# MiNeves00/SR-GAN-FD

Hardware: AMD Instinct MI355X
Metric: SR training images/sec (128->512 x4, f16) (higher is better)
Workload: dtype f16; 1 GPU; BSRGAN RRDBNet x4 generator-only (L1), 23 RRDB, batch 32/GPU, 128->512; global_batch=32, num_rrdb=23, parallelism=dp1

## Files before the change

sr_gan_fd_amd/csrc/conv_igemm.hip:

```cpp
#include "conv_common.hpp"
#include <stdlib.h>
#include <string.h>
#include <utility>
#ifndef SRGANFD_CROSS_MASK
#define SRGANFD_CROSS_MASK 7
#endif
#ifndef SRGANFD_M16_PIPE
#define SRGANFD_M16_PIPE 4
#endif

namespace srganfd {
typedef __attribute__((ext_vector_type(2))) unsigned int u32x2_t;

template <typename T, int KS, int STRIDE, int MR, int WR, int WN, int TS = 1>
struct ConvCfg {
  static constexpr int NWAVES = WR * WN, NTHR = 64 * NWAVES;
  static constexpr int KT = KS * KS;
  static constexpr int TW = 32, TH = WR * MR;
  static constexpr int PR = (TH - 1) * STRIDE + KS;
  static constexpr int PC = (TW - 1) * STRIDE + KS;
  static constexpr int KC = 32;
  static constexpr int E16 = 16 / (int)sizeof(T);
  static constexpr int CPP = KC / E16;
  static constexpr int PIXB = KC * (int)sizeof(T);
// ... 672 lines not shown

template <typename T, int KS, int STRIDE, int MR, int WR, int WN, bool M16 = false, int TS = 1, int EK = -1, bool NT = false>
static int launch_conv(const ConvK& k, int cout, hipStream_t stream) {
  using C = ConvCfg<T, KS, STRIDE, MR, WR, WN, TS>;
  auto kern = conv_igemm_kernel<T, KS, STRIDE, MR, WR, WN, M16, TS, EK, NT>;
  if (g_describe) {
    char ek[8] = "";
    if (EK >= 0) snprintf(ek, sizeof(ek), ",E%d", EK);
    snprintf(g_describe, g_describe_len, "conv_igemm_kernel<%s,KS=%d,S=%d,MR=%d,WR=%d,WN=%d%s%s%s>%s", dtype_name<T>(), KS, STRIDE, MR, WR, WN, M16 ? ",M16" : "", TS > 1 ? ",TS=2" : "", ek,
             k.cls_sh >= 0 ? "[4 classes]" : "");
    return SRGANFD_OK;
  }
  static unsigned long long attr_done = 0;
  if (!g_dry_run) {
    int dev = 0;
    SRGANFD_HIP_CHECK(hipGetDevice(&dev));
    if (!(attr_done >> (dev & 63) & 1ULL)) {
      SRGANFD_HIP_CHECK(hipFuncSetAttribute((const void*)kern, hipFuncAttributeMaxDynamicSharedMemorySize, C::LDS_BYTES));
      attr_done |= 1ULL << (dev & 63);
    }
  }
  ConvK kk = k;
  kk.nNb = cout / C::NB;
  if (k.cls_sh >= 0) {
    if ((KS != 2 && KS != 1) || STRIDE != 1 || sizeof(T) != 2 || (kk.nNb & (kk.nNb - 1)))
      return set_err(SRGANFD_EINVAL, "conv2d: out_classes needs ksize 2 or 1, stride 1 and cout / %d a power of two", C::NB);
    kk.cls_sh = __builtin_ctz((unsigned)kk.nNb);
    kk.nNb *= 4;
  }
  kk.tiles_x = ceil_div(k.Wout, C::TW);
  kk.tiles_y = ceil_div(k.Hout, C::TH);
  const long long nblk = (long long)k.N * kk.tiles_x * kk.tiles_y * kk.nNb;
  if (nblk <= 0 || nblk > 0x7fffffffLL) return set_err(SRGANFD_EINVAL, "conv2d: bad grid %lld", nblk);
  kk.nblocks = (int)nblk;
  kk.m_nNb = div_magic((unsigned)kk.nNb, (unsigned long long)nblk);
  kk.m_tx = div_magic((unsigned)kk.tiles_x, (unsigned long long)nblk);
  kk.m_ty = div_magic((unsigned)kk.tiles_y, (unsigned long long)nblk);
  long long grid = nblk;
  if (EK >= 0 && (EK & SRGANFD_CROSS_MASK) == 0 && sizeof(T) == 2) {
    const long long slots = (long long)conv_device_cus() * C::WG_PER_CU;
    if (slots >= 8 && nblk > slots) grid = slots / 8 * 8;
  }
  SRGANFD_LAUNCH(kern, dim3((unsigned)grid), dim3(C::NTHR), C::LDS_BYTES, stream, kk);
  SRGANFD_HIP_CHECK(hipGetLastError());
  return SRGANFD_OK;
}



int g_mfma16 = 3;
static const bool g_conv_nt = [] { const char* e = getenv("SRGANFD_CONV_NT"); return !(e && e[0] == '0'); }();

bool conv_uses_m16(int dtype, int ksize, int cout) {
  (void)ksize; (void)cout;
  return dtype != SRGANFD_F32;
}

template <typename T>
static int dispatch_conv(const srganfd_conv_args* a, const ConvK& k, hipStream_t s) {
  const bool wide = (a->cout % 64) == 0;
  constexpr bool bf = sizeof(T) == 2;
  if constexpr (bf) {
    if (conv_uses_m16(a->dtype, a->ksize, a->cout)) {
      if (a->ksize == 3 && a->stride == 1) {
        const int ek = (k.fast_epi && !k.y2) ? ((k.r1 ? 1 : 0) | (k.r2 ? 2 : 0) | (k.mask ? 4 : 0)) : -1;
        if (wide) {
          const size_t opix_ = (size_t)a->n * (size_t)k.HoutF * (size_t)k.WoutF;
          if (g_conv_nt && opix_ * (size_t)a->cout_store * 2 >= ((size_t)192 << 20)) {
            if (ek == 0) return launch_conv<T, 3, 1, 2, 4, 2, true, 1, 0, true>(k, a->cout, s);
            if (ek == 4) return launch_conv<T, 3, 1, 2, 4, 2, true, 1, 4, true>(k, a->cout, s);
            if (ek < 0) return launch_conv<T, 3, 1, 2, 4, 2, true, 1, -1, true>(k, a->cout, s);
          }
          if (ek == 0) return launch_conv<T, 3, 1, 2, 4, 2, true, 1, 0>(k, a->cout, s);
          if (ek == 1) return launch_conv<T, 3, 1, 2, 4, 2, true, 1, 1>(k, a->cout, s);
          if (ek == 3) return launch_conv<T, 3, 1, 2, 4, 2, true, 1, 3>(k, a->cout, s);
          if (ek == 4) return launch_conv<T, 3, 1, 2, 4, 2, true, 1, 4>(k, a->cout, s);
          return launch_conv<T, 3, 1, 2, 4, 2, true>(k, a->cout, s);
        }
        if (ek == 0) return launch_conv<T, 3, 1, 2, 8, 1, true, 1, 0>(k, a->cout, s);
        if (ek == 4) return launch_conv<T, 3, 1, 2, 8, 1, true, 1, 4>(k, a->cout, s);
        return launch_conv<T, 3, 1, 2, 8, 1, true>(k, a->cout, s);
      }
      if (a->ksize == 3 && a->stride == 2) return wide ? launch_conv<T, 3, 2, 1, 4, 2, true>(k, a->cout, s) : launch_conv<T, 3, 2, 1, 4, 1, true>(k, a->cout, s);
      if (a->ksize == 2 && a->stride == 1) return wide ? launch_conv<T, 2, 1, 2, 4, 2, true>(k, a->cout, s) : launch_conv<T, 2, 1, 2, 8, 1, true>(k, a->cout, s);
      if (a->ksize == 4 && a->stride == 2) return wide ? launch_conv<T, 4, 2, 1, 4, 2, true, 2>(k, a->cout, s) : launch_conv<T, 4, 2, 1, 4, 1, true>(k, a->cout, s);
      if (a->ksize == 2 && a->stride == 2) return wide ? launch_conv<T, 2, 2, 1, 4, 2, true>(k, a->cout, s) : launch_conv<T, 2, 2, 1, 4, 1, true>(k, a->cout, s);
      if (a->ksize == 1 && a->stride == 1) return launch_conv<T, 1, 1, 2, 4, 1, true>(k, a->cout, s);
      return set_err(SRGANFD_EINVAL, "conv2d: unsupported ksize=%d stride=%d", a->ksize, a->stride);
    }
  }
  if constexpr (bf) {
    return set_err(SRGANFD_EINVAL, "conv2d: the 16-bit kernels run on v_mfma_f32_16x16x32 (ksize %d stride %d has no kernel)", a->ksize, a->stride);
  } else {
    if (a->ksize == 3 && a->stride == 1) return wide ? launch_conv<T, 3, 1, 2, 4, 2>(k, a->cout, s) : launch_conv<T, 3, 1, 2, 8, 1>(k, a->cout, s);
    if (a->ksize == 2 && a->stride == 1) return wide ? launch_conv<T, 2, 1, 2, 4, 2>(k, a->cout, s) : launch_conv<T, 2, 1, 2, 8, 1>(k, a->cout, s);
    if (a->ksize == 4 && a->stride == 2) return launch_conv<T, 4, 2, 1, 4, 1>(k, a->cout, s);
    if (a->ksize == 3 && a->stride == 2) return wide ? launch_conv<T, 3, 2, 1, 4, 2>(k, a->cout, s) : launch_conv<T, 3, 2, 1, 4, 1>(k, a->cout, s);
    if (a->ksize == 2 && a->stride == 2) return wide ? launch_conv<T, 2, 2, 1, 4, 2>(k, a->cout, s) : launch_conv<T, 2, 2, 1, 4, 1>(k, a->cout, s);
    if (a->ksize == 1 && a->stride == 1) return launch_conv<T, 1, 1, 2, 4, 1>(k, a->cout, s);
    return set_err(SRGANFD_EINVAL, "conv2d: unsupported ksize=%d stride=%d", a->ksize, a->stride);
  }
}

int conv_fill_k(const srganfd_conv_args* a, ConvK& k) {
  if (!a || !a->x.ptr || !a->y.ptr || !a->w_packed) return set_err(SRGANFD_EINVAL, "conv2d: null pointer");
  if (a->cin <= 0 || a->cin % 32 || a->cout <= 0 || a->cout % 32 || a->cout_store <= 0 || a->cout_store > a->cout)
    return set_err(SRGANFD_EINVAL, "conv2d: cin=%d cout=%d cout_store=%d (need multiples of 32)", a->cin, a->cout, a->cout_store);
  if (a->n <= 0 || a->h_in <= 0 || a->w_in <= 0 || a->h_out <= 0 || a->w_out <= 0)
    return set_err(SRGANFD_EINVAL, "conv2d: bad dims");
  const int hl = a->h_in << (a->up ? 1 : 0), wl = a->w_in << (a->up ? 1 : 0);
  const bool sub = a->out_sy > 1 || a->out_sx > 1;
  const bool allcls = a->out_classes == 4;
  if (a->out_classes != 0 && a->out_classes != 1 && !allcls) return set_err(SRGANFD_EINVAL, "conv2d: out_classes is 0, 1 or 4");
  if (allcls && (a->out_sy != 2 || a->out_sx != 2 || (a->ksize != 2 && a->ksize != 1) || a->stride != 1 || a->dtype == SRGANFD_F32 || a->up ||
                 (a->class_pad_step != 0 && a->class_pad_step != 1)))
    return set_err(SRGANFD_EINVAL, "conv2d: out_classes = 4 is the 16-bit data gradient of a stride-2 conv (ksize 2 or 1, stride 1, out_sy = out_sx = 2, class_pad_step 0 / 1)");
  if (!sub) {
    const int ho = (hl + 2 * a->pad - a->ksize) / a->stride + 1, wo = (wl + 2 * a->pad - a->ksize) / a->stride + 1;
    if (ho != a->h_out || wo != a->w_out)
      return set_err(SRGANFD_EINVAL, "conv2d: h_out/w_out %dx%d inconsistent with input (expect %dx%d)", a->h_out, a->w_out, ho, wo);
  } else if (a->out_h_full < (a->h_out - 1) * a->out_sy + (allcls ? 1 : a->out_oy) + 1 || a->out_w_full < (a->w_out - 1) * a->out_sx + (allcls ? 1 : a->out_ox) + 1) {
    return set_err(SRGANFD_EINVAL, "conv2d: strided output does not fit the full image");
  }
  const int align = a->dtype == SRGANFD_F32 ? 4 : 8;
  if (a->x.cstride % align || a->x.c0 % align) return set_err(SRGANFD_EINVAL, "conv2d: x view not 16-byte aligned");
  if (a->x.c0 + a->cin > a->x.cstride) return set_err(SRGANFD_EINVAL, "conv2d: x view exceeds buffer channels");
  if (a->y.c0 + a->cout_store > a->y.cstride) return set_err(SRGANFD_EINVAL, "conv2d: y view exceeds buffer channels");
  if ((size_t)a->h_in * a->w_in * (size_t)a->x.cstride >= 0x7fffffffULL)
    return set_err(SRGANFD_EINVAL, "conv2d: one input image is too large for 32-bit element offsets");
  if (a->dtype != SRGANFD_F32 && (size_t)a->h_in * a->w_in * (size_t)a->x.cstride * 2 >= 0x7fffffffULL)
    return set_err(SRGANFD_EINVAL, "conv2d: one input image exceeds the 2 GiB a buffer descriptor's range check can separate from padding");
  const size_t opix = sub ? (size_t)a->out_h_full * a->out_w_full : (size_t)a->h_out * a->w_out;
  auto fits = [&](const srganfd_view& v) { return !v.ptr || opix * (size_t)v.cstride < 0x7fffffffULL; };
  if (!fits(a->y) || !fits(a->y2) || !fits(a->r1) || !fits(a->r2) || !fits(a->mask))
    return set_err(SRGANFD_EINVAL, "conv2d: one output-side image is too large for 32-bit element offsets");
  k.x = a->x.ptr; k.y = a->y.ptr; k.y2 = a->y2.ptr; k.y2C = a->y2.cstride; k.y2_c0 = a->y2.c0;
  k.r1 = a->r1.ptr; k.r2 = a->r2.ptr; k.mask = a->mask.ptr; k.w = a->w_packed;
  k.bias = a->bias; k.alpha_dev = a->alpha_dev;
  k.xC = a->x.cstride; k.x_c0 = a->x.c0; k.yC = a->y.cstride; k.y_c0 = a->y.c0;
  k.r1C = a->r1.cstride; k.r1_c0 = a->r1.c0; k.r2C = a->r2.cstride; k.r2_c0 = a->r2.c0;
  k.mC = a->mask.cstride; k.m_c0 = a->mask.c0;
  {
    const long long ipix = (long long)a->h_in * a->w_in;
    for (const srganfd_view* v : {&a->x, &a->y, &a->y2, &a->r1, &a->r2, &a->mask})
      if (v->ptr && v->planar && (v->c0 % 32 || v->cstride % 32)) return set_err(SRGANFD_EINVAL, "conv2d: a planar view needs c0 and cstride multiples of 32");
    if (a->y.planar && a->y_f32) return set_err(SRGANFD_EINVAL, "conv2d: fp32 output views are NHWC only");
    k.x_ps = a->x.planar ? 32 : a->x.cstride;
    k.x_cs = a->x.planar ? (int)(ipix * 32) : 32;
    k.x_base = a->x.planar ? (a->x.c0 / 32) * k.x_cs : a->x.c0;
    auto out_strides = [&](const srganfd_view& v, int& ps, int& gs) { ps = v.planar ? 32 : v.cstride; gs = v.planar ? (int)(opix * 32) : 32; };
    out_strides(a->y, k.y_ps, k.y_gs); out_strides(a->y2, k.y2_ps, k.y2_gs); out_strides(a->r1, k.r1_ps, k.r1_gs);
    out_strides(a->r2, k.r2_ps, k.r2_gs); out_strides(a->mask, k.m_ps, k.m_gs);
  }
  k.N = a->n; k.Hin = a->h_in; k.Win = a->w_in; k.up = a->up ? 1 : 0; k.pad_y = sub ? a->pad_y : a->pad; k.pad_x = sub ? a->pad_x : a->pad;
  k.osy = sub ? a->out_sy : 1; k.osx = sub ? a->out_sx : 1; k.ooy = sub ? a->out_oy : 0; k.oox = sub ? a->out_ox : 0;
  k.HoutF = sub ? a->out_h_full : a->h_out; k.WoutF = sub ? a->out_w_full : a->w_out;
  k.Hout = a->h_out; k.Wout = a->w_out; k.nChunks = a->cin / 32; k.nNb = 0; k.cls_sh = allcls ? 0 : -1; k.cls_pad = allcls ? a->class_pad_step : 0; k.cout_store = a->cout_store;
  k.tiles_x = k.tiles_y = 0;
  k.alpha = a->alpha; k.slope = a->slope; k.post_scale = a->post_scale; k.r1s = a->r1_scale; k.r2s = a->r2_scale;
  k.mask_slope = a->mask_slope; k.act = a->act; k.y_f32 = a->y_f32 ? 1 : 0;
  auto aligned = [&](const srganfd_view& v) { return !v.ptr || (v.cstride % align == 0 && v.c0 % align == 0 && ((uintptr_t)v.ptr & 15) == 0); };
  k.fast_epi = (!a->y_f32 && a->cout_store == a->cout && aligned(a->y) && aligned(a->y2) && aligned(a->r1) && aligned(a->r2) && aligned(a->mask)) ? 1 : 0;
  return SRGANFD_OK;
}

int conv2d_impl(const srganfd_conv_args* a, hipStream_t stream) {
  ConvK k;
  {
    const int rc = conv_fill_k(a, k);
    if (rc != SRGANFD_OK) return rc;
  }
  if (a->dtype == SRGANFD_BF16) return dispatch_conv<bf16_t>(a, k, stream);
  if (a->dtype == SRGANFD_F16) return dispatch_conv<f16_t>(a, k, stream);
  if (a->dtype == SRGANFD_F32) return dispatch_conv<float>(a, k, stream);
  return set_err(SRGANFD_EINVAL, "conv2d: bad dtype %d", a->dtype);
}

}
```

sr_gan_fd_amd/csrc/pack.hip:

```cpp
#include "common.hpp"

namespace srganfd {

__global__ __launch_bounds__(256) void pack_kernel(const srganfd_pack_job* __restrict__ jobs, const float* __restrict__ params,
                                                   const float* __restrict__ scalars, char* __restrict__ packed) {
  const srganfd_pack_job& J = jobs[blockIdx.y];
  const int KT = J.ksize * J.ksize;
  const long long total = (long long)KT * J.k * J.n;
  const int nChunks = J.k >> 5;
  for (long long e = (long long)blockIdx.x * 256 + threadIdx.x; e < total; e += (long long)gridDim.x * 256) {
    int lane, s, k_in, within = (int)(e & 1023);
    long long blk = e >> 10;
    const int tap = (int)(blk % KT); blk /= KT;
    const int chunk = (int)(blk % nChunks);
    const int ntile = (int)(blk / nChunks);
    int n_in = -1;
    if (J.dtype != SRGANFD_F32 && J.layout == 1) {
      const int j = within & 7; lane = (within >> 3) & 63; s = within >> 9;
      k_in = 8 * (lane >> 4) + j;
      n_in = 16 * s + (lane & 15);
    } else if (J.dtype != SRGANFD_F32) {
      const int j = within & 7; lane = (within >> 3) & 63; s = within >> 9;
      k_in = 16 * s + 8 * (lane >> 5) + j;
    } else {
      lane = within & 63; s = within >> 6;
      k_in = 2 * s + (lane >> 5);
    }
    const int k = chunk * 32 + k_in, n = ntile * 32 + (n_in >= 0 ? n_in : (lane & 31));
    float v = 0.f;
    for (int g = 0; g < J.nseg; ++g) {
      const srganfd_pack_seg& S = J.seg[g];
      if (k >= S.k_lo && k < S.k_lo + S.k_len) {
        const int kk = k - S.k_lo;
        int co, ci, t;
        int KTs = KT;
        if (!S.transposed) { co = n + S.co_off; ci = kk + S.ci_off; t = tap; }
        else if (S.transposed == 1) { co = kk + S.co_off; ci = n + S.ci_off; t = KT - 1 - tap; }
        else if (S.transposed < 6) {
          const int py = (S.transposed - 2) >> 1, px = (S.transposed - 2) & 1, ta = tap >> 1, tb = tap & 1;
          const int ty = py ? 2 - 2 * ta : 3 - 2 * ta, tx = px ? 2 - 2 * tb : 3 - 2 * tb;
          co = kk + S.co_off; ci = n + S.ci_off; t = ty * 4 + tx; KTs = 16;
        } else if (S.transposed < 10) {
          const int py = (S.transposed - 6) >> 1, px = (S.transposed - 6) & 1, ta = tap >> 1, tb = tap & 1;
          const int ty = py ? (ta ? 0 : 2) : (ta ? -1 : 1), tx = px ? (tb ? 0 : 2) : (tb ? -1 : 1);
          co = kk + S.co_off; ci = n + S.ci_off; KTs = 9;
          t = ty * 3 + tx;
          if (ty < 0 || tx < 0) co = S.co_src;
        } else {
          const int ab = S.transposed - 10;
          co = kk + S.co_off; ci = n + S.ci_off; t = ab; KTs = 4;
        }
        if (co < S.co_src && ci < S.ci_src) {
          v = params[S.src_off + ((long long)co * S.ci_src + ci) * KTs + t] * S.scale;
          if (S.scale_off >= 0) v *= scalars[S.scale_off];
        }
        break;
      }
    }
    if (J.dtype == SRGANFD_BF16) ((bf16_t*)(packed + J.dst_off))[e] = f2bf(v);
    else if (J.dtype == SRGANFD_F16) ((f16_t*)(packed + J.dst_off))[e] = (f16_t)v;
    else ((float*)(packed + J.dst_off))[e] = v;
  }
}

int pack_weights_impl(const srganfd_pack_job* jobs_dev, int njobs, long long max_elems, const float* params,
                      const float* scalars, void* packed, hipStream_t stream) {
  if (!jobs_dev || njobs <= 0 || max_elems <= 0 || !params || !packed) return set_err(SRGANFD_EINVAL, "pack_weights: bad args");
  long long gx = (max_elems + 255) / 256;
  if (gx > 4096) gx = 4096;
  SRGANFD_LAUNCH(pack_kernel, dim3((unsigned)gx, (unsigned)njobs), dim3(256), 0, stream, jobs_dev, params, scalars, (char*)packed);
  SRGANFD_HIP_CHECK(hipGetLastError());
  return SRGANFD_OK;
}

}
```

sr_gan_fd_amd/engine.py:

```python
from __future__ import annotations

import ctypes as C
import os
import weakref
from typing import Dict, List, Optional, Sequence, Tuple

import torch
from torch import Tensor, nn

from . import _abi as A
from . import ops
from . import profiling

_ENGINES: "weakref.WeakKeyDictionary[nn.Module, object]" = weakref.WeakKeyDictionary()


def _require_gpu(x: Tensor) -> None:
    if not x.is_cuda and not A.DRY_RUN:
        raise A.SrganfdError("sr_gan_fd_amd runs on MI355X only: input tensor is not on a GPU (no CPU fallback)")
    A.lib()


def check_channels(what: str, x: Tensor, channels: int) -> None:
    if x.dim() != 4 or x.shape[1] != channels:
# ... 50 lines not shown
                for p, o, n, s in zip(self.params, self.offsets, self.numels, self.shapes):
                    f[o:o + n].copy_(p.detach().reshape(-1).to(device=device, dtype=torch.float32))
                    p.data = f[o:o + n].view(s)
            self.flat = f
            self.version += 1
        return f

    def touch(self) -> None:
        self.version += 1

    def signature(self) -> tuple:
        return (self.flat.data_ptr(), self.flat._version, self.version, tuple(p._version for p in self.params))

    def stale(self, pk: dict) -> bool:
        sig = self.signature()
        if pk.get("seen") != sig:
            pk["seen"] = sig
            return True
        return False

    def new_grad(self, device) -> Tensor:
        if self.total == sum(self.numels):
            return torch.empty(self.total, dtype=torch.float32, device=device)
        return torch.zeros(self.total, dtype=torch.float32, device=device)

    def grad_views(self, flat_grad: Tensor) -> List[Tensor]:
        return [flat_grad[o:o + n].view(s) for o, n, s in zip(self.offsets, self.numels, self.shapes)]


class _Shape:
    pass


class PlanCache:

    def __init__(self, cap: int = 8, cap_pinned: int = 2):
        from collections import OrderedDict
        self.d: "OrderedDict[tuple, tuple]" = OrderedDict()
        self.cap, self.cap_pinned = cap, cap_pinned

    def get(self, key):
        v = self.d.get(key)
        if v is None:
            return None
        self.d.move_to_end(key)
        return v[0]

    def put(self, key, sp, pinned: bool = False) -> None:
        self.d[key] = (sp, pinned)
        self.d.move_to_end(key)
        for want_pinned, cap in ((False, self.cap), (True, self.cap_pinned)):
            keys = [k for k, (_, pin) in self.d.items() if pin == want_pinned]
            for k in keys[:max(0, len(keys) - cap)]:
                del self.d[k]

    def __setitem__(self, key, sp) -> None:
        self.put(key, sp)

    def __len__(self) -> int:
        return len(self.d)

    def __contains__(self, key) -> bool:
        return key in self.d

    def clear(self) -> None:
        self.d.clear()


class TrunkEngine:

    def __init__(self, owner: nn.Module, rdbs: Sequence[nn.Module], rrdb: bool, full: bool):
        self.owner = owner
        self.rdbs = list(rdbs)
        self.rrdb = rrdb
        self.full = full
        self.R = len(self.rdbs)
        c5 = self.rdbs[0].conv5.weight
        self.Cc = c5.shape[0]
        self.G = self.rdbs[0].conv1.weight.shape[0]
        if self.Cc % 32 or self.G % 32:
            raise A.SrganfdError("channels and growth_channels must be multiples of 32 for the MFMA path")
        self.Ccat = self.Cc + 4 * self.G
        self.unshuffle = 1
        if full:
            self.n_up = owner.n_upsample()
            self.in_ch = owner.conv1.weight.shape[1]
            self.out_ch = owner.conv4.weight.shape[0]
            self.unshuffle = getattr(owner, "unshuffle", 1)
        self.fp = FlatParams(list(owner.named_parameters()))
        self.shapes = PlanCache()
        self.packed: Dict[int, dict] = {}
        self.token = 0
        self._rdb_prefix = self._find_prefixes()

    def _find_prefixes(self) -> List[str]:
        names = {id(m): n for n, m in self.owner.named_modules()}
        out = []
        for r in self.rdbs:
            n = names[id(r)]
            out.append(n + "." if n else "")
        return out

    def _poff(self, name: str) -> int:
        return self.fp.off(name)

    def _build_pack(self, dtc: int, device) -> dict:
        Cc, G, Ccat = self.Cc, self.G, self.Ccat
        jobs, offs, cur = [], {}, 0

        def add(key, ksize, k, n, segs):
            nonlocal cur
            offs[key] = cur
            jobs.append(ops.pack_job(cur, dtc, ksize, k, n, segs))
            cur += (ops.packed_bytes(dtc, ksize, k, n) + 255) // 256 * 256

        def fwd(key, wname, co, ci):
            add(key, 3, ops.pad32(ci), ops.pad32(co), [dict(src_off=self._poff(wname), co_src=co, ci_src=ci, k_len=ops.pad32(ci))])

        def bwd(key, wname, co, ci):
            add(key, 3, ops.pad32(co), ops.pad32(ci), [dict(src_off=self._poff(wname), co_src=co, ci_src=ci, k_len=ops.pad32(co), transposed=1)])

        for i, pre in enumerate(self._rdb_prefix):
            for k in range(1, 6):
                cin, cout = Cc + (k - 1) * G, (Cc if k == 5 else G)
                fwd(("f", i, k), f"{pre}conv{k}.weight", cout, cin)
            s5 = 0.2 * (0.2 if (self.rrdb and i % 3 == 2) else 1.0)
            dyoff = {5: 0, 4: Cc, 3: Cc + G, 2: Cc + 2 * G, 1: Cc + 3 * G}
            for step in range(5):
                c_lo = Cc + (3 - step) * G if step < 4 else 0
                n = G if step < 4 else Cc
                kdim = Cc + step * G
                segs = []
                for j in range(5, 4 - step, -1):
                    cin_j, cout_j = Cc + (j - 1) * G, (Cc if j == 5 else G)
                    segs.append(dict(src_off=self._poff(f"{pre}conv{j}.weight"), co_src=cout_j, ci_src=cin_j, k_lo=dyoff[j],
                                     k_len=cout_j, ci_off=c_lo, transposed=1, scale=(s5 if j == 5 else 1.0)))
                add(("b", i, step), 3, kdim, n, segs)
        if self.full:
            fwd(("f", "conv1"), "conv1.weight", Cc, self.in_ch)
            for nm in ["conv2"] + [f"upsampling{u}.0" for u in range(1, self.n_up + 1)] + ["conv3.0"]:
                fwd(("f", nm), nm + ".weight", Cc, Cc)
                bwd(("b", nm), nm + ".weight", Cc, Cc)
            fwd(("f", "conv4"), "conv4.weight", self.out_ch, Cc)
            bwd(("b", "conv4"), "conv4.weight", self.out_ch, Cc)
        table = ops.PackTable(jobs, device)
        buf = torch.empty(cur, dtype=torch.uint8, device=device)
        return dict(table=table, offs=offs, buf=buf)

    def _ensure_packed(self, dtc: int, device) -> dict:
        flat = self.fp.sync(device)
        pk = self.packed.get(dtc)
        if pk is None or pk["buf"].device != device or pk.get("flat_ptr") != flat.data_ptr():
            pk = self._build_pack(dtc, device)
            pk["flat_ptr"] = flat.data_ptr()
            self.packed[dtc] = pk
        if self.fp.stale(pk):
            pk["table"].run(flat, pk["buf"])
        return pk

    def _plan(self, N: int, H: int, W: int, dt: torch.dtype, dtc: int, device, train: bool, pk: dict) -> _Shape:
        key = (N, H, W, dtc, train, str(device), pk["buf"].data_ptr(), self.fp.flat.data_ptr())
        sp = self.shapes.get(key)
        if sp is not None:
            return sp
        sp = _Shape()
        Cc, G, Ccat, R = self.Cc, self.G, self.Ccat, self.R
        flat = self.fp.flat
        fptr = flat.data_ptr()
        wptr = pk["buf"].data_ptr()

        def new(*shape, dtype=dt):
            return torch.empty(*shape, dtype=dtype, device=device)

        if train:
            cat = sp.cat = [new(N, H, W, Ccat) for _ in range(R + 1)]
            catb = lambda i: cat[i]
        else:
            cat = sp.cat = [new(N, H, W, Ccat) for _ in range(min(R + 1, 5))]
            catb = lambda i: cat[0] if i == 0 else cat[1 + (i - 1) % 4]
        sp.catb = catb
        V = A.view
        sp.planar = 1 if (self.full and os.environ.get("SRGANFD_PLANAR", "1") != "0") else 0
        VC = lambda t, c0=0: A.view(t, c0=c0, planar=sp.planar)

        def bias(name):
            return fptr + 4 * self._poff(name)

        fw = []
        if self.full:
            s = 1 << self.n_up
            sp.thin_i, sp.thin_o = ops.thin_ok(dtc, Cc, self.in_ch), ops.thin_ok(dtc, Cc, self.out_ch)
            cin1 = ops.pad32(self.in_ch)
            sp.xin = new(N, H, W, 4 if sp.thin_i else cin1)
            sp.f0 = new(N, H, W, Cc)
            sp.ups = [new(N, H << u, W << u, Cc) for u in range(1, self.n_up + 1)]
            sp.c3 = new(N, H * s, W * s, Cc)
            sp.srp = new(N, H * s, W * s, 4, dtype=torch.float32)
            if sp.thin_i:
                fw.append(ops.ThinLaunch("thin_in", ops.thin_args(dtc, N, H, W, self.in_ch, bias("conv1.weight"), VC(catb(0)), w_big_is_cout=True,
                                                                  bias=bias("conv1.bias"), thin=sp.xin)))
            else:
                fw.append(ops.conv_args(dtc, V(sp.xin), VC(catb(0)), wptr + pk["offs"][("f", "conv1")], N, H, W, cin1, Cc, bias=bias("conv1.bias")))
        for i, pre in enumerate(self._rdb_prefix):
            ci = catb(i)
            blk = []
            for k in range(1, 5):
                blk.append(ops.conv_args(dtc, VC(ci), VC(ci, c0=Cc + (k - 1) * G), wptr + pk["offs"][("f", i, k)], N, H, W, Cc + (k - 1) * G, G,
                                         bias=bias(f"{pre}conv{k}.bias"), act=A.ACT_LRELU, slope=0.2))
            last = self.rrdb and i % 3 == 2
            kw = dict(post_scale=0.04, r1=VC(ci), r1_scale=0.2, r2=VC(catb(i - 2)), r2_scale=1.0) if last else \
                dict(post_scale=0.2, r1=VC(ci), r1_scale=1.0)
            blk.append(ops.conv_args(dtc, VC(ci), VC(catb(i + 1)), wptr + pk["offs"][("f", i, 5)], N, H, W, Ccat, Cc,
                                     bias=bias(f"{pre}conv5.bias"), **kw))
            fw.extend(ops.dense_chain_or_launches(blk, device) if (Cc, G) == (64, 32) else blk)
        if self.full:
            tout = catb(R)
            fw.append(ops.conv_args(dtc, VC(tout), V(sp.f0), wptr + pk["offs"][("f", "conv2")], N, H, W, Cc, Cc, bias=bias("conv2.bias"),
                                    r1=VC(catb(0)), r1_scale=1.0))
            src, h, w = sp.f0, H, W
            for u in range(1, self.n_up + 1):
                nm = f"upsampling{u}.0"
                fw.append(ops.conv_args(dtc, V(src), V(sp.ups[u - 1]), wptr + pk["offs"][("f", nm)], N, h, w, Cc, Cc, up=1,
                                        bias=bias(nm + ".bias"), act=A.ACT_LRELU, slope=0.2))
                src, h, w = sp.ups[u - 1], h * 2, w * 2
            fw.append(ops.conv_args(dtc, V(src), V(sp.c3), wptr + pk["offs"][("f", "conv3.0")], N, h, w, Cc, Cc, bias=bias("conv3.0.bias"),
                                    act=A.ACT_LRELU, slope=0.2))
            if sp.thin_o:
                fw.append(ops.ThinLaunch("thin_out", ops.thin_args(dtc, N, h, w, self.out_ch, bias("conv4.weight"), V(sp.c3), w_big_is_cout=False,
                                                                   bias=bias("conv4.bias"), thin_out=sp.srp, thin_out_pitch=4)))
            else:
                fw.append(ops.conv_args(dtc, V(sp.c3), V(sp.srp), wptr + pk["offs"][("f", "conv4")], N, h, w, Cc, 32, cout_store=self.out_ch,
                                        bias=bias("conv4.bias"), y_f32=True))
            sp.hs, sp.ws = h, w
        sp.fw = fw
        sp.N, sp.H, sp.W, sp.dt, sp.dtc, sp.device = N, H, W, dt, dtc, device
        if train:
            self._plan_backward(sp, pk)
        self.shapes.put(key, sp, pinned=train)
        return sp

    def _plan_backward(self, sp: _Shape, pk: dict) -> None:
        N, H, W, dt, dtc, device = sp.N, sp.H, sp.W, sp.dt, sp.dtc, sp.device
        Cc, G, Ccat, R = self.Cc, self.G, self.Ccat, self.R
        wptr = pk["buf"].data_ptr()
        V = A.view
        VC = lambda t, c0=0: A.view(t, c0=c0, planar=sp.planar)
        VD = VC

        def new(*shape, dtype=dt):
            return torch.empty(*shape, dtype=dtype, device=device)

        sp.dy = [new(N, H, W, Ccat) for _ in range(4)]
        sp.dx0 = new(N, H, W, Cc)
        dyb = lambda i: sp.dy[i % 4]
        bw: List[tuple] = []
        ws_bytes = 0

        def wplan(n, h, w, xch, dych, convs, up=0):
            nonlocal ws_bytes
            p = ops.WgradPlan(device, dtc, n, h, w, xch, dych, convs, up=up)
            ws_bytes = max(ws_bytes, p.workspace_bytes)
            return p

        if self.full:
            s = 1 << self.n_up
            hs, ws_ = sp.hs, sp.ws
            sp.dsrp = new(N, hs, ws_, 4 if sp.thin_o else 32)
            sp.gA = new(N, hs, ws_, Cc)
            fptr = self.fp.flat.data_ptr()
            if sp.thin_i or sp.thin_o:
                sp.thin_ws = torch.empty(ops.thin_wgrad_workspace_bytes(), dtype=torch.uint8, device=device)
            sp.gB = new(N, hs, ws_, Cc)
            sp.glo = [new(N, H << u, W << u, Cc) for u in range(0, self.n_up)]

            def one(name, cout, cin, dw_only=False):
                return [dict(cin=ops.pad32(cin), cout=ops.pad32(cout), dw_off=self._poff(name + ".weight"), db_off=self._poff(name + ".bias"),
                             co_dst=cout, ci_dst=cin)]
            if sp.thin_o:
                w4 = fptr + 4 * self._poff("conv4.weight")
                bw.append(("thin", ops.ThinLaunch("thin_wgrad", ops.thin_args(dtc, N, hs, ws_, self.out_ch, w4, V(sp.c3), w_big_is_cout=False, thin=sp.dsrp),
                                                  dw_off=self._poff("conv4.weight"), db_off=self._poff("conv4.bias"), ws=sp.thin_ws)))
                bw.append(("thin", ops.ThinLaunch("thin_in", ops.thin_args(dtc, N, hs, ws_, self.out_ch, w4, V(sp.gA), w_big_is_cout=False, flip=True,
                                                                           mask=V(sp.c3), mask_slope=0.2, thin=sp.dsrp))))
            else:
                bw.append(("wgrad", wplan(N, hs, ws_, Cc, 32, one("conv4", self.out_ch, Cc)), V(sp.c3), V(sp.dsrp), 0))
                bw.append(("conv", ops.conv_args(dtc, V(sp.dsrp), V(sp.gA), wptr + pk["offs"][("b", "conv4")], N, hs, ws_, 32, Cc, mask=V(sp.c3), mask_slope=0.2)))
            src3 = sp.ups[-1] if self.n_up else sp.f0
            bw.append(("wgrad", wplan(N, hs, ws_, Cc, Cc, one("conv3.0", Cc, Cc)), V(src3), V(sp.gA), 0))
            if self.n_up:
                bw.append(("conv", ops.conv_args(dtc, V(sp.gA), V(sp.gB), wptr + pk["offs"][("b", "conv3.0")], N, hs, ws_, Cc, Cc, mask=V(src3), mask_slope=0.2)))
            else:
                bw.append(("conv", ops.conv_args(dtc, V(sp.gA), V(sp.gB), wptr + pk["offs"][("b", "conv3.0")], N, hs, ws_, Cc, Cc)))
            cur, other = sp.gB, sp.gA
            for u in range(self.n_up, 0, -1):
                nm = f"upsampling{u}.0"
                hin, win = H << (u - 1), W << (u - 1)
                xin_t = sp.ups[u - 2] if u >= 2 else sp.f0
                npx = N * (hin * 2) * (win * 2)
                cur_v = V(cur.view(-1)[: npx * Cc].view(N, hin * 2, win * 2, Cc))
                oth_v = V(other.view(-1)[: npx * Cc].view(N, hin * 2, win * 2, Cc))
                bw.append(("wgrad", wplan(N, hin, win, Cc, Cc, one(nm, Cc, Cc), up=1), V(xin_t), cur_v, 0))
                bw.append(("conv", ops.conv_args(dtc, cur_v, oth_v, wptr + pk["offs"][("b", nm)], N, hin * 2, win * 2, Cc, Cc)))
                glo = sp.glo[u - 1]
                bw.append(("call", (lambda a=oth_v, b=V(glo), hh=hin, ww=win: A.check(
                    A.lib().srganfd_resample(0, a, b, dtc, N, hh, ww, Cc, A.stream_ptr()), "nearest_bwd"))))
                if u >= 2:
                    bw.append(("call", (lambda d=V(glo), act=V(xin_t), npx2=N * hin * win: A.check(
                        A.lib().srganfd_lrelu_bwd(d, act, A.NULL_VIEW, d, dtc, npx2, Cc, 0.2, A.stream_ptr()), "lrelu_bwd"))))
                    cur, other = glo, sp.gA
                else:
                    cur = glo
            d_f0 = cur if self.n_up else sp.gB
            sp.d_f0 = d_f0
            bw.append(("wgrad", wplan(N, H, W, Cc, Cc, one("conv2", Cc, Cc)), VC(sp.catb(R)), V(d_f0), 0))
            bw.append(("conv", ops.conv_args(dtc, V(d_f0), VD(dyb(R - 1)), wptr + pk["offs"][("b", "conv2")], N, H, W, Cc, Cc)))
            bw.append(("ready", self._poff("conv2.weight"), self.fp.total))
        rdb_names = ["conv%d" % k for k in range(1, 6)]
        plans = {}
        for i in range(R - 1, -1, -1):
            pre = self._rdb_prefix[i]
            last = self.rrdb and i % 3 == 2
            first = self.rrdb and i % 3 == 0
            s_out = 0.2 if last else 1.0
            s5 = 0.2 * s_out
            ci, di = sp.catb(i), dyb(i)
            if s5 not in plans:
                base = self._poff(pre + "conv1.weight")
                convs = []
                for k in range(1, 6):
                    cin, cout = Cc + (k - 1) * G, (Cc if k == 5 else G)
                    convs.append(dict(ci_lo=0, cin=cin, co_lo=(0 if k == 5 else Cc + (4 - k) * G), cout=cout,
                                      dw_off=self._poff(pre + f"conv{k}.weight") - base, db_off=self._poff(pre + f"conv{k}.bias") - base,
                                      co_dst=cout, ci_dst=cin, alpha=(s5 if k == 5 else 1.0)))
                plans[s5] = wplan(N, H, W, Ccat, Ccat, convs)
            blk = []
            for step in range(4):
                kdim = Cc + step * G
                blk.append(ops.conv_args(dtc, VD(di), VD(di, c0=Cc + step * G), wptr + pk["offs"][("b", i, step)], N, H, W, kdim, G,
                                         mask=VC(ci, c0=Cc + (3 - step) * G), mask_slope=0.2))
            dst = VD(dyb(i - 1)) if i > 0 else V(sp.dx0)
            kw = dict(r1=VD(di), r1_scale=s_out)
            if first:
                kw.update(r2=VD(dyb(i + 2)), r2_scale=1.0)
            blk.append(ops.conv_args(dtc, VD(di), dst, wptr + pk["offs"][("b", i, 4)], N, H, W, Ccat, Cc, **kw))
            chain = ops.dense_chain_or_launches(blk, sp.device) if (Cc, G) == (64, 32) else blk
            wg = ("wgrad", plans[s5], VC(ci), VD(di), self._poff(pre + "conv1.weight"), i)
            fence = [("fence", i + 3)] if i > 0 else []
            ready = [("ready", self._poff(pre + "conv1.weight"), self._poff("conv2.weight"))] if self.full and R >= 4 and i == R // 2 else []
            if len(chain) == 1:
                bw.extend(fence + [("chain", chain[0]), wg] + ready)
            else:
                bw.extend([("conv", a_) for a_ in blk[:4]] + [wg] + ready + fence + [("conv", blk[4])])
        if self.full:
            bw.append(("call", (lambda x=V(sp.d_f0), y=V(sp.dx0): A.check(
                A.lib().srganfd_axpby(x, y, dtc, N * H * W, Cc, 1.0, 1.0, A.stream_ptr()), "axpby"))))
            if sp.thin_i:
                bw.append(("thin", ops.ThinLaunch("thin_wgrad", ops.thin_args(dtc, N, H, W, self.in_ch, self.fp.flat.data_ptr() + 4 * self._poff("conv1.weight"),
                                                                              V(sp.dx0), w_big_is_cout=True, thin=sp.xin),
                                                  dw_off=self._poff("conv1.weight"), db_off=self._poff("conv1.bias"), ws=sp.thin_ws)))
            else:
                cin1 = ops.pad32(self.in_ch)
                convs = [dict(cin=cin1, cout=Cc, dw_off=self._poff("conv1.weight"), db_off=self._poff("conv1.bias"), co_dst=Cc, ci_dst=self.in_ch)]
                bw.append(("wgrad", wplan(N, H, W, cin1, Cc, convs), V(sp.xin), V(sp.dx0), 0))
        covered = min([it[1] for it in bw if it[0] == "ready"], default=self.fp.total)
        bw.append(("ready", 0, covered))
        sp.bw = bw
        sp.wg_ws = torch.empty(ws_bytes, dtype=torch.uint8, device=device)
        dense_ws = max((p_.workspace_bytes for p_ in plans.values()), default=0)
        sp.wg_ws4 = [torch.empty(dense_ws, dtype=torch.uint8, device=device) for _ in range(_BATCH_REDUCE)] if (dense_ws and _BATCH_REDUCE > 1) else None

    def trunk_size(self, shape) -> Tuple[int, int, int]:
        shape = tuple(shape)
        u = self.unshuffle
        want_c = self.in_ch // (u * u) if self.full else self.Cc
        what = "generator" if self.full else "dense block"
        if len(shape) != 4:
            raise A.SrganfdError(f"{what} expects a 4-D (N, {want_c}, H, W) input, got shape {shape}")
        N, c, H, W = shape
        if c != want_c:
            raise A.SrganfdError(f"{what} expects (N, {want_c}, H, W) inputs, got shape {shape}")
        if H % u or W % u:
            raise A.SrganfdError(f"generator with PixelUnshuffle({u}) expects H and W divisible by {u}: (N, {want_c}, {u}k, {u}m), "
                                 f"got shape {shape}")
        return N, H // u, W // u

    def output_shape(self, shape) -> Tuple[int, int, int, int]:
        N, H, W = self.trunk_size(shape)
        if not self.full:
            return (N, self.Cc, H, W)
        return (N, self.out_ch, H << self.n_up, W << self.n_up)

# ... 213 lines not shown
```

sr_gan_fd_amd/profiling.py:

```python
from __future__ import annotations

from typing import Dict, List, Optional

import torch

REC: Optional["Recorder"] = None


class Recorder:

    def __init__(self, every: int = 7):
        self.items: List[tuple] = []
        self.every = max(1, every)
        self.count: Dict[str, int] = {}
        self.work: Dict[str, list] = {}

    def bracket(self, label: str, work, fn) -> None:
        flops, nbytes = work if isinstance(work, tuple) else (work, 0.0)
        n = self.count.get(label, 0)
        self.count[label] = n + 1
        w = self.work.setdefault(label, [0.0, 0.0])
        w[0] += flops
        w[1] += nbytes
        if n % self.every:
            fn()
            return
        e0, e1 = torch.cuda.Event(enable_timing=True), torch.cuda.Event(enable_timing=True)
        e0.record()
        fn()
        e1.record()
        self.items.append((label, flops, nbytes, e0, e1))


def enable(every: int = 7) -> Recorder:
    global REC
    REC = Recorder(every)
    return REC


def disable() -> None:
    global REC
    REC = None


def conv_label(a) -> str:
    lab = getattr(a, "_kernel_label", None)
    if lab is None:
        import ctypes as C
        from . import _abi as A
        buf = C.create_string_buffer(160)
        A.check(A.lib().srganfd_conv2d_describe(C.byref(a), buf, 160), "conv2d_describe")
        lab = a._kernel_label = buf.value.decode()
    return lab


def conv_flops(a) -> float:
    return 2.0 * a.n * a.h_out * a.w_out * a.ksize * a.ksize * a.cin * a.cout_store * (4 if a.out_classes == 4 else 1)


def conv_work(a) -> tuple:
    es = 4 if a.dtype == 1 else 2
    pin = a.n * a.h_in * a.w_in * a.cin * es
    pout = a.n * a.h_out * a.w_out * a.cout_store * (4 if a.out_classes == 4 else 1)
    nb = pin + pout * (4 if a.y_f32 else es)
    for v in (a.r1, a.r2, a.mask, a.y2):
        if v.ptr:
            nb += pout * es
    return conv_flops(a), float(nb)


def summary(rec: Recorder) -> Dict[str, dict]:
    torch.cuda.synchronize()
    agg: Dict[str, dict] = {}
    for label, flops, nbytes, e0, e1 in rec.items:
        d = agg.setdefault(label, {"launches": 0, "ms": 0.0, "flop": 0.0, "bytes": 0.0, "timed_launches": 0})
        d["timed_launches"] += 1
        d["ms"] += e0.elapsed_time(e1)
        d["flop"] += flops
        d["bytes"] += nbytes
    for label, d in agg.items():
        d["launches"] = rec.count[label]
    for d in agg.values():
        d["avg_us"] = round(d["ms"] * 1e3 / d["timed_launches"], 2)
        d["tflops"] = round(d["flop"] / (d["ms"] * 1e-3) / 1e12, 1) if d["ms"] > 0 else 0.0
        d["gbps"] = round(d["bytes"] / (d["ms"] * 1e-3) / 1e9, 1) if d["ms"] > 0 else 0.0
        d["flop_per_byte"] = round(d["flop"] / d["bytes"], 1) if d["bytes"] > 0 else None
        scale = d["launches"] / d["timed_launches"]
        d["ms"] = round(d["ms"] * scale, 3)
    for label, d in agg.items():
        d["flop"] = float(f"{rec.work[label][0]:.6g}")
        d["bytes"] = float(f"{rec.work[label][1]:.6g}")
    return agg


MEASURED_READ_GBPS = 5600.0


def roofline(rec: Recorder, peak_tflops: float, peak_gbps: float = 8000.0) -> dict:
    import re
    per_label = summary(rec)
    agg: Dict[str, dict] = {}
    for lab, v in per_label.items():
        fam = re.sub(r",E\d+", "", lab)
        d = agg.setdefault(fam, {"launches": 0, "ms": 0.0, "flop": 0.0, "bytes": 0.0, "kinds": {}})
        d["launches"] += v["launches"]; d["ms"] += v["ms"]; d["flop"] += v["flop"]; d["bytes"] += v["bytes"]
        d["kinds"][lab] = {"launches": v["launches"], "avg_us": v["avg_us"]}
    for d in agg.values():
        d["avg_us"] = round(d["ms"] * 1e3 / d["launches"], 2) if d["launches"] else 0.0
        d["tflops"] = round(d["flop"] / (d["ms"] * 1e-3) / 1e12, 1) if d["ms"] > 0 else 0.0
        d["gbps"] = round(d["bytes"] / (d["ms"] * 1e-3) / 1e9, 1) if d["ms"] > 0 else 0.0
        d["flop_per_byte"] = round(d["flop"] / d["bytes"], 1) if d["bytes"] > 0 else None
    label, d = max(agg.items(), key=lambda kv: kv[1]["ms"])
    ridge = peak_tflops * 1e12 / (peak_gbps * 1e9)
    ai = d["flop_per_byte"]
    hbm = ai is not None and ai < ridge
    out = {"bound": "hbm" if hbm else "mfma", "kernel": label}
    if hbm:
        out.update(achieved=d["gbps"], peak=peak_gbps, unit="GB/s", frac=round(d["gbps"] / peak_gbps, 4))
    else:
        out.update(achieved=d["tflops"], peak=peak_tflops, unit="TFLOP/s", frac=round(d["tflops"] / peak_tflops, 4))
    if len(d["kinds"]) > 1:
        out["kinds"] = d["kinds"]
    slab, sv = max(per_label.items(), key=lambda kv: kv[1]["ms"])
    tot_ms = sum(v["ms"] for v in per_label.values())
    out["largest_symbol"] = {"kernel": slab, "avg_us": sv["avg_us"], "launches": sv["launches"], "tflops": sv["tflops"],
                             "mfma_frac": round(sv["tflops"] / peak_tflops, 4), "share_of_bracketed_kernel_time": round(sv["ms"] / tot_ms, 4) if tot_ms > 0 else None}
    out.update(traffic=None, avg_launch_us=d["avg_us"], launches=d["launches"],
               flop_per_launch=float(f"{d['flop'] / d['launches']:.6g}"),
               bytes_per_launch=float(f"{d['bytes'] / d['launches']:.6g}"), flop_per_byte=ai, ridge_flop_per_byte=round(ridge, 1),
               mfma_frac=round(d["tflops"] / peak_tflops, 4), hbm_frac=round(d["gbps"] / peak_gbps, 4),
               hbm_measured_read_gbps=MEASURED_READ_GBPS, hbm_frac_of_measured=round(d["gbps"] / MEASURED_READ_GBPS, 4))
    return out
```

Before: 539.6 img/s.

## Fold nearest-x2 upsample into parity-decomposed 2x2 convs and 4x4 stride-2 dgrad

Replaces each nearest-x2 upsample followed by a 3x3 conv with four sub-pixel 2x2 convs, whose weights are summed at pack time from the 3x3 taps for each output parity. Where possible these run as a single out_classes=4 launch that works on the low-resolution input. The backward data gradient becomes one 4x4 stride-2 conv with folded weights and a fused leaky-ReLU mask, replacing the conv, nearest-resample reduction and lrelu_bwd kernels. A non-temporal-store variant of the 2x2 kernel is added for large outputs. This removes the 2.25x redundant MACs of convolving the upsampled image and several full-resolution memory passes, at the cost of new pack modes and layout complexity.

```diff
diff --git a/sr_gan_fd_amd/csrc/conv_igemm.hip b/sr_gan_fd_amd/csrc/conv_igemm.hip
--- a/sr_gan_fd_amd/csrc/conv_igemm.hip
+++ b/sr_gan_fd_amd/csrc/conv_igemm.hip
@@ -778,7 +778,11 @@
         return launch_conv<T, 3, 1, 2, 8, 1, true>(k, a->cout, s);
       }
       if (a->ksize == 3 && a->stride == 2) return wide ? launch_conv<T, 3, 2, 1, 4, 2, true>(k, a->cout, s) : launch_conv<T, 3, 2, 1, 4, 1, true>(k, a->cout, s);
-      if (a->ksize == 2 && a->stride == 1) return wide ? launch_conv<T, 2, 1, 2, 4, 2, true>(k, a->cout, s) : launch_conv<T, 2, 1, 2, 8, 1, true>(k, a->cout, s);
+      if (a->ksize == 2 && a->stride == 1) {
+        if (wide && g_conv_nt && k.cls_sh >= 0 && a->bias && (size_t)a->n * (size_t)k.HoutF * (size_t)k.WoutF * (size_t)a->cout_store * 2 >= ((size_t)192 << 20))
+          return launch_conv<T, 2, 1, 2, 4, 2, true, 1, -1, true>(k, a->cout, s);
+        return wide ? launch_conv<T, 2, 1, 2, 4, 2, true>(k, a->cout, s) : launch_conv<T, 2, 1, 2, 8, 1, true>(k, a->cout, s);
+      }
       if (a->ksize == 4 && a->stride == 2) return wide ? launch_conv<T, 4, 2, 1, 4, 2, true, 2>(k, a->cout, s) : launch_conv<T, 4, 2, 1, 4, 1, true>(k, a->cout, s);
       if (a->ksize == 2 && a->stride == 2) return wide ? launch_conv<T, 2, 2, 1, 4, 2, true>(k, a->cout, s) : launch_conv<T, 2, 2, 1, 4, 1, true>(k, a->cout, s);
       if (a->ksize == 1 && a->stride == 1) return launch_conv<T, 1, 1, 2, 4, 1, true>(k, a->cout, s);
@@ -810,7 +814,8 @@
   if (a->out_classes != 0 && a->out_classes != 1 && !allcls) return set_err(SRGANFD_EINVAL, "conv2d: out_classes is 0, 1 or 4");
   if (allcls && (a->out_sy != 2 || a->out_sx != 2 || (a->ksize != 2 && a->ksize != 1) || a->stride != 1 || a->dtype == SRGANFD_F32 || a->up ||
                  (a->class_pad_step != 0 && a->class_pad_step != 1)))
-    return set_err(SRGANFD_EINVAL, "conv2d: out_classes = 4 is the 16-bit data gradient of a stride-2 conv (ksize 2 or 1, stride 1, out_sy = out_sx = 2, class_pad_step 0 / 1)");
+    return set_err(SRGANFD_EINVAL, "conv2d: out_classes = 4 is the 16-bit data gradient of a stride-2 conv or the forward of a nearest-x2 + 3x3 conv "
+                                   "(ksize 2 or 1, stride 1, up 0, out_sy = out_sx = 2, class_pad_step 0 / 1)");
   if (!sub) {
     const int ho = (hl + 2 * a->pad - a->ksize) / a->stride + 1, wo = (wl + 2 * a->pad - a->ksize) / a->stride + 1;
     if (ho != a->h_out || wo != a->w_out)
diff --git a/sr_gan_fd_amd/csrc/pack.hip b/sr_gan_fd_amd/csrc/pack.hip
--- a/sr_gan_fd_amd/csrc/pack.hip
+++ b/sr_gan_fd_amd/csrc/pack.hip
@@ -32,8 +32,9 @@
       const srganfd_pack_seg& S = J.seg[g];
       if (k >= S.k_lo && k < S.k_lo + S.k_len) {
         const int kk = k - S.k_lo;
-        int co, ci, t;
+        int co, ci, t = 0;
         int KTs = KT;
+        int ym = 0, xm = 0;
         if (!S.transposed) { co = n + S.co_off; ci = kk + S.ci_off; t = tap; }
         else if (S.transposed == 1) { co = kk + S.co_off; ci = n + S.ci_off; t = KT - 1 - tap; }
         else if (S.transposed < 6) {
@@ -46,12 +47,31 @@
           co = kk + S.co_off; ci = n + S.ci_off; KTs = 9;
           t = ty * 3 + tx;
           if (ty < 0 || tx < 0) co = S.co_src;
-        } else {
+        } else if (S.transposed < 14) {
           const int ab = S.transposed - 10;
           co = kk + S.co_off; ci = n + S.ci_off; t = ab; KTs = 4;
+        } else if (S.transposed < 18) {
+          const int py = (S.transposed - 14) >> 1, px = (S.transposed - 14) & 1, ta = tap >> 1, tb = tap & 1;
+          co = n + S.co_off; ci = kk + S.ci_off; KTs = 9;
+          ym = py ? (ta ? 4 : 3) : (ta ? 6 : 1);
+          xm = px ? (tb ? 4 : 3) : (tb ? 6 : 1);
+        } else {
+          const int u = tap >> 2, w = tap & 3;
+          co = kk + S.co_off; ci = n + S.ci_off; KTs = 9;
+          ym = (0x1364 >> (4 * u)) & 7;
+          xm = (0x1364 >> (4 * w)) & 7;
         }
         if (co < S.co_src && ci < S.ci_src) {
-          v = params[S.src_off + ((long long)co * S.ci_src + ci) * KTs + t] * S.scale;
+          const float* src = params + S.src_off + ((long long)co * S.ci_src + ci) * KTs;
+          if (ym) {
+            float sum = 0.f;
+            for (int ty = 0; ty < 3; ++ty)
+              for (int tx = 0; tx < 3; ++tx)
+                if ((ym >> ty) & (xm >> tx) & 1) sum += src[ty * 3 + tx];
+            v = sum * S.scale;
+          } else {
+            v = src[t] * S.scale;
+          }
           if (S.scale_off >= 0) v *= scalars[S.scale_off];
         }
         break;
diff --git a/sr_gan_fd_amd/engine.py b/sr_gan_fd_amd/engine.py
--- a/sr_gan_fd_amd/engine.py
+++ b/sr_gan_fd_amd/engine.py
@@ -156,6 +156,7 @@
             raise A.SrganfdError("channels and growth_channels must be multiples of 32 for the MFMA path")
         self.Ccat = self.Cc + 4 * self.G
         self.unshuffle = 1
+        self.up_parity = os.environ.get("SRGANFD_UPSAMPLE_PARITY", "1") != "0"
         if full:
             self.n_up = owner.n_upsample()
             self.in_ch = owner.conv1.weight.shape[1]
@@ -177,6 +178,9 @@
 
     def _poff(self, name: str) -> int:
         return self.fp.off(name)
+
+    def _parity(self, dtc: int) -> bool:
+        return self.full and self.up_parity and dtc != A.F32
 
     def _build_pack(self, dtc: int, device) -> dict:
         Cc, G, Ccat = self.Cc, self.G, self.Ccat
@@ -212,7 +216,14 @@
                 add(("b", i, step), 3, kdim, n, segs)
         if self.full:
             fwd(("f", "conv1"), "conv1.weight", Cc, self.in_ch)
-            for nm in ["conv2"] + [f"upsampling{u}.0" for u in range(1, self.n_up + 1)] + ["conv3.0"]:
+            ups = [f"upsampling{u}.0" for u in range(1, self.n_up + 1)]
+            for nm in ["conv2"] + ups + ["conv3.0"]:
+                if nm in ups and self._parity(dtc):
+                    src = self._poff(nm + ".weight")
+                    for c in range(4):
+                        add(("fc", nm, c), 2, Cc, Cc, [dict(src_off=src, co_src=Cc, ci_src=Cc, k_len=Cc, transposed=14 + c)])
+                    add(("b4", nm), 4, Cc, Cc, [dict(src_off=src, co_src=Cc, ci_src=Cc, k_len=Cc, transposed=18)])
+                    continue
                 fwd(("f", nm), nm + ".weight", Cc, Cc)
                 bwd(("b", nm), nm + ".weight", Cc, Cc)
             fwd(("f", "conv4"), "conv4.weight", self.out_ch, Cc)
@@ -294,8 +305,11 @@
             src, h, w = sp.f0, H, W
             for u in range(1, self.n_up + 1):
                 nm = f"upsampling{u}.0"
-                fw.append(ops.conv_args(dtc, V(src), V(sp.ups[u - 1]), wptr + pk["offs"][("f", nm)], N, h, w, Cc, Cc, up=1,
-                                        bias=bias(nm + ".bias"), act=A.ACT_LRELU, slope=0.2))
+                if self._parity(dtc):
+                    fw.extend(self._up_forward(dtc, pk, V(src), V(sp.ups[u - 1]), N, h, w, bias(nm + ".bias"), nm))
+                else:
+                    fw.append(ops.conv_args(dtc, V(src), V(sp.ups[u - 1]), wptr + pk["offs"][("f", nm)], N, h, w, Cc, Cc, up=1,
+                                            bias=bias(nm + ".bias"), act=A.ACT_LRELU, slope=0.2))
                 src, h, w = sp.ups[u - 1], h * 2, w * 2
             fw.append(ops.conv_args(dtc, V(src), V(sp.c3), wptr + pk["offs"][("f", "conv3.0")], N, h, w, Cc, Cc, bias=bias("conv3.0.bias"),
                                     act=A.ACT_LRELU, slope=0.2))
@@ -312,6 +326,22 @@
             self._plan_backward(sp, pk)
         self.shapes.put(key, sp, pinned=train)
         return sp
+
+    def _up_forward(self, dtc: int, pk: dict, x: A.View, y: A.View, N: int, h: int, w: int, bias: int, nm: str) -> List[A.ConvArgs]:
+        Cc, O, wptr = self.Cc, pk["offs"], pk["buf"].data_ptr()
+        one = ops.class4_ok(dtc, Cc, [O[("fc", nm, c)] for c in range(4)], ops.packed_bytes(dtc, 2, Cc, Cc))
+        out = []
+        for par in range(1 if one else 4):
+            py, px = par >> 1, par & 1
+            a = ops.conv_args(dtc, x, y, wptr + O[("fc", nm, par)], N, h, w, Cc, Cc, ksize=2, stride=1, pad=0, bias=bias, act=A.ACT_LRELU, slope=0.2)
+            a.h_out, a.w_out = h, w
+            a.out_sy, a.out_sx, a.out_oy, a.out_ox = 2, 2, py, px
+            a.out_h_full, a.out_w_full = 2 * h, 2 * w
+            a.pad_y, a.pad_x = (1, 1) if one else (1 - py, 1 - px)
+            a.out_classes, a.class_pad_step = (4, 1) if one else (0, 0)
+            a._label_tag = " nearest-x2 fwd"
+            out.append(a)
+        return out
 
     def _plan_backward(self, sp: _Shape, pk: dict) -> None:
         N, H, W, dt, dtc, device = sp.N, sp.H, sp.W, sp.dt, sp.dtc, sp.device
@@ -374,13 +404,20 @@
                 cur_v = V(cur.view(-1)[: npx * Cc].view(N, hin * 2, win * 2, Cc))
                 oth_v = V(other.view(-1)[: npx * Cc].view(N, hin * 2, win * 2, Cc))
                 bw.append(("wgrad", wplan(N, hin, win, Cc, Cc, one(nm, Cc, Cc), up=1), V(xin_t), cur_v, 0))
-                bw.append(("conv", ops.conv_args(dtc, cur_v, oth_v, wptr + pk["offs"][("b", nm)], N, hin * 2, win * 2, Cc, Cc)))
                 glo = sp.glo[u - 1]
-                bw.append(("call", (lambda a=oth_v, b=V(glo), hh=hin, ww=win: A.check(
-                    A.lib().srganfd_resample(0, a, b, dtc, N, hh, ww, Cc, A.stream_ptr()), "nearest_bwd"))))
+                if self._parity(dtc):
+                    a = ops.conv_args(dtc, cur_v, V(glo), wptr + pk["offs"][("b4", nm)], N, hin * 2, win * 2, Cc, Cc, ksize=4, stride=2, pad=1,
+                                      mask=V(xin_t) if u >= 2 else A.NULL_VIEW, mask_slope=0.2)
+                    a._label_tag = " nearest-x2 dgrad"
+                    bw.append(("conv", a))
+                else:
+                    bw.append(("conv", ops.conv_args(dtc, cur_v, oth_v, wptr + pk["offs"][("b", nm)], N, hin * 2, win * 2, Cc, Cc)))
+                    bw.append(("call", (lambda a=oth_v, b=V(glo), hh=hin, ww=win: A.check(
+                        A.lib().srganfd_resample(0, a, b, dtc, N, hh, ww, Cc, A.stream_ptr()), "nearest_bwd"))))
+                    if u >= 2:
+                        bw.append(("call", (lambda d=V(glo), act=V(xin_t), npx2=N * hin * win: A.check(
+                            A.lib().srganfd_lrelu_bwd(d, act, A.NULL_VIEW, d, dtc, npx2, Cc, 0.2, A.stream_ptr()), "lrelu_bwd"))))
                 if u >= 2:
-                    bw.append(("call", (lambda d=V(glo), act=V(xin_t), npx2=N * hin * win: A.check(
-                        A.lib().srganfd_lrelu_bwd(d, act, A.NULL_VIEW, d, dtc, npx2, Cc, 0.2, A.stream_ptr()), "lrelu_bwd"))))
                     cur, other = glo, sp.gA
                 else:
                     cur = glo
diff --git a/sr_gan_fd_amd/profiling.py b/sr_gan_fd_amd/profiling.py
--- a/sr_gan_fd_amd/profiling.py
+++ b/sr_gan_fd_amd/profiling.py
@@ -50,7 +50,7 @@
         from . import _abi as A
         buf = C.create_string_buffer(160)
         A.check(A.lib().srganfd_conv2d_describe(C.byref(a), buf, 160), "conv2d_describe")
-        lab = a._kernel_label = buf.value.decode()
+        lab = a._kernel_label = buf.value.decode() + getattr(a, "_label_tag", "")
     return lab
 
 
```

Measured after the change: 548.6 img/s, median of 6. 1.02x the previous value.
